# UM-Applied-Algorithms-Lab/AWRY

Hardware: AMD Instinct MI355X
Metric: k-mer count queries/sec (parallel_count, random 31-mers, index resident in HBM) (higher is better)
Workload: dtype u64

## Files before the change

### awry_amd/csrc/kernels_nt2_kmer.hip.h

```cpp
#pragma once

namespace awry {

__device__ __forceinline__ void tally_flush(unsigned long long* __restrict__ tally, uint32_t t_probe, uint32_t t_step, uint32_t t_blk) {
  atomicAdd(&tally[0], (unsigned long long)t_probe);
  atomicAdd(&tally[1], (unsigned long long)t_step);
  atomicAdd(&tally[2], (unsigned long long)t_blk);
}

template <bool USE_SEED, bool TALLY>
__global__ __launch_bounds__(256) void count_nt2_quad_kernel(DevIndex ix, const uint64_t* __restrict__ queries, uint64_t n, int L,
                                                             uint64_t* __restrict__ counts, unsigned long long* __restrict__ tally) {
  const int l = threadIdx.x & 3;
  const uint64_t nquads = ((uint64_t)gridDim.x * blockDim.x) >> 2;
  uint64_t q = ((uint64_t)blockIdx.x * blockDim.x + threadIdx.x) >> 2;
  const uint64_t* __restrict__ blocks = ix.blocks;
  const SeedEntry* __restrict__ seed = ix.seed;
  const int k = USE_SEED ? ix.seed_k : 1;
  const uint32_t cA = (uint32_t)ix.prefix_sums[1], cC = (uint32_t)ix.prefix_sums[2], cG = (uint32_t)ix.prefix_sums[3],
                 cN = (uint32_t)ix.prefix_sums[4], cT = (uint32_t)ix.prefix_sums[5], cEnd = (uint32_t)ix.prefix_sums[6];

  bool have = q < n;
  uint64_t w = have ? queries[q] : 0;
  bool fresh = true;
  uint32_t sp = 1, ep = 0;
  int i = 0;
  uint32_t t_probe = 0, t_step = 0, t_blk = 0;

  while (__any(have)) {
    if (have) {
      if (fresh) {
        if (USE_SEED) {
          const uint64_t sidx = ((w >> (2 * (L - k))) & ((1ull << (2 * k)) - 1));
          kmer_seed_start(seed[sidx], w, L - k, ix.seed_pos, sp, ep, i);
          if (TALLY) t_probe++;
        }
        if (!USE_SEED || i < 0) {
          const uint32_t c = (uint32_t)(w >> (2 * (L - 1))) & 3u;
          sp = c == 0 ? cA : (c == 1 ? cC : (c == 2 ? cG : cT));
          ep = (c == 0 ? cC : (c == 1 ? cG : (c == 2 ? cN : cEnd))) - 1;
          i = L - 1;
        }
        fresh = false;
      } else {
        i--;
        const uint32_t c = (uint32_t)(w >> (2 * i)) & 3u;
        const uint32_t cl = c == 0 ? cA : (c == 1 ? cC : (c == 2 ? cG : cT));
        if (TALLY) { t_step++; t_blk += ((sp - 1) >> 8) == (ep >> 8) ? 1u : 2u; }
        quad_step(blocks, cl, sp, ep, c, l);
      }
      if (sp > ep || i == 0) {
        if (l == 0) counts[q] = sp > ep ? 0ull : (uint64_t)(ep - sp) + 1ull;
        q += nquads;
        have = q < n;
        if (have) w = queries[q];
        fresh = true;
      }
    }
  }
  if (TALLY && l == 0) {
    tally_flush(tally, t_probe, t_step, t_blk);
  }
}

constexpr int TALLY_DEEP_STEP = 10;

template <bool USE_SEED, bool TALLY, bool VERIFY>
__global__ __launch_bounds__(256) void count_nt2_quad4_kernel(DevIndex ix, const uint64_t* __restrict__ queries, uint64_t n, int L,
                                                              uint64_t* __restrict__ counts, unsigned long long* __restrict__ tally) {
  const int lane = threadIdx.x & 63, l = lane & 3;
  const uint64_t nquads = ((uint64_t)gridDim.x * blockDim.x) >> 2;
  const uint64_t ngroups = (n + 3) >> 2;
  uint64_t m = ((uint64_t)blockIdx.x * blockDim.x + threadIdx.x) >> 2;
  const uint64_t* __restrict__ blocks = ix.blocks;
  const SeedEntry* __restrict__ seed = ix.seed;
  const int k = USE_SEED ? ix.seed_k : 1;
  const int verify_after = (int)ix.verify_after;
  const uint32_t cA = (uint32_t)ix.prefix_sums[1], cC = (uint32_t)ix.prefix_sums[2], cG = (uint32_t)ix.prefix_sums[3],
                 cN = (uint32_t)ix.prefix_sums[4], cT = (uint32_t)ix.prefix_sums[5], cEnd = (uint32_t)ix.prefix_sums[6];
  const int kshift = 2 * (L - k);
  const uint64_t kmask = (1ull << (2 * k)) - 1;
  bool have = m < ngroups;
  uint64_t wq = (have && 4 * m + l < n) ? queries[4 * m + l] : 0;
  uint64_t eq = 0;
  if (USE_SEED && have) { const SeedEntry e0 = seed[((wq >> kshift) & kmask)]; eq = (uint64_t)e0.sp | ((uint64_t)e0.cnt << 32); }
  uint64_t wq_next = (m + nquads < ngroups && 4 * (m + nquads) + l < n) ? queries[4 * (m + nquads) + l] : 0;
  int nvalid = have ? (int)(n - 4 * m < 4 ? n - 4 * m : 4) : 0;
  int t = 0;
  bool fresh = true;
  uint64_t w = 0, res = 0;
  uint32_t sp = 1, ep = 0;
  int i = 0, steps_done = 0;
  int mode = 0, vj = 0;
  uint32_t vhits = 0, vp = 0;
  uint32_t t_probe = 0, t_step = 0, t_blk = 0, t_vsa = 0, t_vtxt = 0, t_deep = 0;

  while (__any(have)) {
    if (have) {
      bool finished = false;
      uint64_t out_count = 0;
      if (!VERIFY || mode == 0) {
        if (fresh) {
          w = __shfl(wq, (lane & ~3) | t, 64);
          if (USE_SEED) {
            const uint64_t ev = __shfl(eq, (lane & ~3) | t, 64);
            kmer_seed_start(SeedEntry{(uint32_t)ev, (uint32_t)(ev >> 32)}, w, L - k, ix.seed_pos, sp, ep, i);
            if (TALLY) t_probe++;
          }
          if (!USE_SEED || i < 0) {
            const uint32_t c = (uint32_t)(w >> (2 * (L - 1))) & 3u;
            sp = c == 0 ? cA : (c == 1 ? cC : (c == 2 ? cG : cT));
            ep = (c == 0 ? cC : (c == 1 ? cG : (c == 2 ? cN : cEnd))) - 1;
            i = L - 1;
          }
          steps_done = 0;
          fresh = false;
        } else {
          i--;
          const uint32_t c = (uint32_t)(w >> (2 * i)) & 3u;
          const uint32_t cl = c == 0 ? cA : (c == 1 ? cC : (c == 2 ? cG : cT));
          if (TALLY) {
            const uint32_t nb = ((sp - 1) >> 8) == (ep >> 8) ? 1u : 2u;
            t_step++;
            t_blk += nb;
            if (steps_done >= TALLY_DEEP_STEP) t_deep += nb;
          }
          quad_step(blocks, cl, sp, ep, c, l);
          steps_done++;
        }
        if (sp > ep || i == 0) {
          finished = true;
          out_count = sp > ep ? 0ull : (uint64_t)(ep - sp) + 1ull;
        } else if (VERIFY) {
          const uint32_t cnt = ep - sp + 1u;
          if (verify_now(cnt, i, steps_done, verify_after)) { mode = 1; vj = 0; vhits = 0; }
        }
      } else if (mode == 1) {
        vp = ix.dense_sa[sp + (uint32_t)vj];
        if (TALLY) t_vsa++;
        if (vp >= (uint32_t)i) mode = 2;
        else vj++;
      } else {
        const uint32_t bad = quad_sum(verify_part(ix.text4, (uint64_t)vp - (uint64_t)i, i, 0, l, w));
        if (TALLY) t_vtxt++;
        if (!bad) vhits++;
        vj++;
        mode = 1;
      }
      if (VERIFY && mode == 1 && vj > (int)(ep - sp)) { finished = true; out_count = vhits; }
      if (finished) {
        if (l == t) res = out_count;
        t++;
        fresh = true;
        mode = 0;
        if (t == nvalid) {
          if (l < nvalid) counts[4 * m + l] = res;
          m += nquads;
          have = m < ngroups;
          t = 0;
          nvalid = have ? (int)(n - 4 * m < 4 ? n - 4 * m : 4) : 0;
          wq = wq_next;
          if (USE_SEED && have) { const SeedEntry e0 = seed[((wq >> kshift) & kmask)]; eq = (uint64_t)e0.sp | ((uint64_t)e0.cnt << 32); }
          wq_next = (m + nquads < ngroups && 4 * (m + nquads) + l < n) ? queries[4 * (m + nquads) + l] : 0;
        }
      }
    }
  }
  if (TALLY && l == 0) {
    tally_flush(tally, t_probe, t_step, t_blk);
    atomicAdd(&tally[5], (unsigned long long)t_deep);
    if (VERIFY) {
      atomicAdd(&tally[3], (unsigned long long)t_vsa);
      atomicAdd(&tally[4], (unsigned long long)t_vtxt);
    }
  }
}

constexpr int VMULTI = 4;
constexpr int LCX_LANE_ROWS = 4;
constexpr int LCX_TAIL_MAX = 16;

struct Nt2Survivors {
  uint64_t* w;
  uint64_t* range;
  uint32_t* q;
  uint32_t* count;
  uint64_t cap;
  uint32_t* lf_count = nullptr;
};

template <bool TALLY, bool VERIFY>
__device__ __forceinline__ unsigned probe_block(const DevIndex& ix, const uint64_t* __restrict__ queries, uint64_t n, int L,
                                                uint64_t* __restrict__ counts, const Nt2Survivors& sv,
                                                unsigned long long* __restrict__ tally) {
  __shared__ unsigned int s_count;
  constexpr int VQ = 192;
  __shared__ uint64_t s_vw[VERIFY ? 4 : 1][VQ];
  __shared__ uint32_t s_vsp[VERIFY ? 4 : 1][VQ];
  __shared__ uint32_t s_vq[VERIFY ? 4 : 1][VQ];
  __shared__ uint8_t s_vn[VERIFY ? 4 : 1][VQ];
  if (threadIdx.x == 0) s_count = 0;
  if (blockIdx.x == 0 && threadIdx.x == 0 && sv.lf_count) *sv.lf_count = 0;
  __syncthreads();
  const int lane = threadIdx.x & 63, wv_id = threadIdx.x >> 6;
  const SeedEntry* __restrict__ seed = ix.seed;
  const int k = ix.seed_k, i0 = L - k, kshift = 2 * (L - k);
  const uint64_t kmask = (1ull << (2 * k)) - 1;
  const uint64_t stride = (uint64_t)gridDim.x * blockDim.x;
  const uint64_t lane_lt = (1ull << lane) - 1;
  const uint64_t region = (uint64_t)blockIdx.x * sv.cap;
  const bool pos = VERIFY && ix.seed_pos;
  const int cx = (int)ix.ctx_extra, clen = SEED_CTX_LEN + cx;
  const bool verify = VERIFY && (i0 >= 3 || (pos && i0 >= 1));
  const bool lcx = VERIFY && ix.lcx_key != nullptr && i0 >= 1;
  int vcount = 0;
  uint32_t t_vsa = 0, t_vtxt = 0, t_lcx = 0;
  auto drain = [&](int base, int cnt) {
    uint64_t w[2];
    uint32_t q[2], sp[2], nc[2], vp[2];
    bool on[2];
#pragma unroll
    for (int h = 0; h < 2; h++) {
      const int s = base + lane + 64 * h;
      on[h] = lane + 64 * h < cnt;
      w[h] = on[h] ? s_vw[VERIFY ? wv_id : 0][s] : 0;
      q[h] = on[h] ? s_vq[VERIFY ? wv_id : 0][s] : 0;
      sp[h] = on[h] ? s_vsp[VERIFY ? wv_id : 0][s] : 0;
      nc[h] = on[h] ? s_vn[VERIFY ? wv_id : 0][s] : 0;
      vp[h] = sp[h];
      if (on[h] && !(nc[h] & 0x80u) && !(pos && nc[h] == 1u)) { vp[h] = ix.dense_sa[sp[h]]; if (TALLY) t_vsa++; }
    }
#pragma unroll
    for (int h = 0; h < 2; h++) {
      if (!on[h]) continue;
      uint64_t value = 0;
      if (nc[h] & 0x80u) {
        const uint64_t want = (w[h] & ((1ull << (2 * i0)) - 1)) << (64 - 2 * i0);
        const uint32_t rows = nc[h] & 0x7Fu;
        const uint64_t* __restrict__ kp = ix.lcx_key + sp[h];
        const uint64_t k0 = kp[0], k1 = kp[1], k2 = rows > 2u ? kp[2] : ~want, k3 = rows > 3u ? kp[3] : ~want;
        const int sh = 64 - 2 * i0;
        value = (((k0 ^ want) >> sh) == 0) + (((k1 ^ want) >> sh) == 0) + (((k2 ^ want) >> sh) == 0) + (((k3 ^ want) >> sh) == 0);
        if (TALLY) t_lcx++;
        counts[q[h]] = value;
        continue;
      }
      for (uint32_t c = 0; c < nc[h]; c++) {
        const uint32_t p = c ? ix.dense_sa[sp[h] + c] : vp[h];
        if (TALLY && c) t_vsa++;
        if (p >= (uint32_t)i0) {
          if (TALLY) t_vtxt++;
          value += verify_part(ix.text4, (uint64_t)p - (uint64_t)i0, i0, 0, 0, w[h]) ? 0ull : 1ull;
        }
      }
      counts[q[h]] = value;
    }
  };
  constexpr int NQ = 4;
  for (uint64_t wbase = (uint64_t)blockIdx.x * blockDim.x + (threadIdx.x & ~63u); wbase < n; wbase += NQ * stride) {
    uint64_t qv[NQ], wv[NQ];
    SeedEntry ev[NQ];
#pragma unroll
    for (int h = 0; h < NQ; h++) {
      qv[h] = wbase + lane + (uint64_t)h * stride;
      wv[h] = qv[h] < n ? queries[qv[h]] : 0;
    }
#pragma unroll
    for (int h = 0; h < NQ; h++) {
      ev[h] = SeedEntry{1u, 0u};
      if (qv[h] < n) ev[h] = seed_probe(seed + ((wv[h] >> kshift) & kmask));
    }
#pragma unroll
    for (int h = 0; h < NQ; h++) {
      const bool valid = qv[h] < n;
      const uint64_t q = qv[h], w = wv[h];
      const SeedEntry e = ev[h];
      const uint32_t cnt = seed_cnt(e);
      bool survivor = false, queued = false, lcx_q = false;
      uint64_t value = 0;
      if (valid) {
        if (cnt == SEED_CNT_SAT) survivor = true;
        else if (cnt == 0u) value = 0;
        else if (i0 == 0) value = cnt;
        else if (cnt == 1u && pos && seed_has_ctx(e) && i0 <= clen) {
          value = (w & ((1ull << (2 * i0)) - 1)) == (seed_full_ctx(e, cx) >> (2 * (clen - i0))) ? 1ull : 0ull;
        } else if (cnt == 1u && pos && seed_has_ctx(e)) {
          queued = ((w >> (2 * (i0 - clen))) & ((1ull << (2 * clen)) - 1)) == seed_full_ctx(e, cx);
        } else if (cnt == 1u) {
          const uint32_t nc = (uint32_t)(w >> (2 * (i0 - 1))) & 3u;
          survivor = seed_sym(e) == (int)(nc == 3u ? 5u : nc + 1u);
          if (verify && survivor) { queued = true; survivor = false; }
        } else if (lcx && !(e.cnt & (SEED_LCX_NONE | SEED_LCX_TAIL)) && cnt <= (uint32_t)LCX_LANE_ROWS) {
          queued = true;
          lcx_q = true;
        } else if (lcx && !(e.cnt & SEED_LCX_NONE)) {
          survivor = true;
        } else if (verify && cnt <= (uint32_t)VMULTI && (int)(3u * cnt) <= i0 + 2) {
          queued = true;
        } else survivor = true;
        if (!queued) counts[q] = value;
      }
      if (VERIFY) {
        const uint64_t qm = __ballot(queued);
        if (qm) {
          if (queued) {
            const int s = vcount + (int)__popcll(qm & lane_lt);
            s_vw[wv_id][s] = w;
            s_vsp[wv_id][s] = cnt == 1u && pos ? seed_position(e, cx) : e.sp;
            s_vq[wv_id][s] = (uint32_t)q;
            s_vn[wv_id][s] = (uint8_t)(cnt | (lcx_q ? 0x80u : 0u));
          }
          vcount += (int)__popcll(qm);
          __builtin_amdgcn_wave_barrier();
          if (vcount >= 128) {
            vcount -= 128;
            drain(vcount, 128);
            __builtin_amdgcn_wave_barrier();
          }
        }
      }
      const uint64_t sm = __ballot(survivor);
      if (sm) {
        unsigned int slot0 = 0;
        if (lane == 0) slot0 = atomicAdd(&s_count, (unsigned int)__popcll(sm));
        slot0 = __shfl(slot0, 0, 64);
        if (survivor) {
          const uint64_t s = region + slot0 + (uint64_t)__popcll(sm & lane_lt);
          sv.w[s] = w;
          sv.range[s] = (uint64_t)e.sp | ((uint64_t)(cnt | (e.cnt & (SEED_LCX_NONE | SEED_LCX_TAIL))) << 32);
          sv.q[s] = (uint32_t)q;
        }
      }
    }
  }
  if (VERIFY && vcount > 0) drain(0, vcount);
  if (TALLY) {
    if (blockIdx.x == 0 && threadIdx.x == 0) atomicAdd(&tally[0], (unsigned long long)n);
    if (VERIFY && (t_vsa | t_vtxt | t_lcx)) {
      atomicAdd(&tally[3], (unsigned long long)t_vsa);
      atomicAdd(&tally[4], (unsigned long long)t_vtxt);
      atomicAdd(&tally[6], (unsigned long long)t_lcx);
    }
  }
  __syncthreads();
  return s_count;
}

template <bool TALLY, bool VERIFY>
__global__ __launch_bounds__(256) void count_nt2_probe_kernel(DevIndex ix, const uint64_t* __restrict__ queries, uint64_t n, int L,
                                                              uint64_t* __restrict__ counts, Nt2Survivors sv,
                                                              unsigned long long* __restrict__ tally) {
  const unsigned ns = probe_block<TALLY, VERIFY>(ix, queries, n, L, counts, sv, tally);
  if (threadIdx.x == 0) sv.count[blockIdx.x] = ns;
}

template <bool TALLY, bool VERIFY, bool TABLE = false>
__device__ __forceinline__ void resume_block_list(const DevIndex& ix, const Nt2Survivors& sv, uint64_t region, uint64_t ns, int L,
                                                  uint64_t* __restrict__ counts, unsigned long long* __restrict__ tally, bool allow_lcx,
                                                  uint64_t r_start, uint64_t r_stride) {
  const int l = threadIdx.x & 3;
  uint64_t r = r_start;
  const uint64_t* __restrict__ blocks = ix.blocks;
  const int k = ix.seed_k;
  const int verify_after = (int)ix.verify_after;
  const bool lcx = VERIFY && ix.lcx_key != nullptr && allow_lcx;
  const uint32_t cA = (uint32_t)ix.prefix_sums[1], cC = (uint32_t)ix.prefix_sums[2], cG = (uint32_t)ix.prefix_sums[3],
                 cN = (uint32_t)ix.prefix_sums[4], cT = (uint32_t)ix.prefix_sums[5], cEnd = (uint32_t)ix.prefix_sums[6];
  bool have = r < ns, fresh = true;
  uint64_t w = 0;
  uint32_t sp = 1, ep = 0, qidx = 0;
  int i = 0, steps_done = 0;
  int mode = 0, vj = 0;
  uint32_t vhits = 0, vp = 0;
  uint32_t ub_a = 0, ub_b = 0;
  const LcxRefs lq{vp, vhits, ub_a, ub_b, vj};
  uint32_t t_step = 0, t_blk = 0, t_vsa = 0, t_vtxt = 0, t_lcx = 0, t_rp = 0;
  uint64_t nx_w = 0, nx_rg = 0;
  uint32_t nx_q = 0;
  if (have) { nx_w = sv.w[region + r]; nx_rg = sv.range[region + r]; nx_q = sv.q[region + r]; }
  while (__any(have)) {
    if (have) {
      bool finished = false;
      uint64_t out_count = 0;
      if (mode == 0) {
        if (fresh) {
          w = nx_w;
          const uint64_t rg = nx_rg;
          qidx = nx_q;
          if (r + r_stride < ns) { nx_w = sv.w[region + r + r_stride]; nx_rg = sv.range[region + r + r_stride]; nx_q = sv.q[region + r + r_stride]; }
          const uint32_t cf = (uint32_t)(rg >> 32), cnt = cf & SEED_CNT_SAT;
          steps_done = 0;
          fresh = false;
          if (qidx == 0xFFFFFFFFu) {
            sp = 1u; ep = 0u; i = 0;
          } else if (cnt == SEED_CNT_SAT) {
            const uint32_t c = (uint32_t)(w >> (2 * (L - 1))) & 3u;
            sp = c == 0 ? cA : (c == 1 ? cC : (c == 2 ? cG : cT));
            ep = (c == 0 ? cC : (c == 1 ? cG : (c == 2 ? cN : cEnd))) - 1;
            i = L - 1;
          } else {
            sp = (uint32_t)rg;
            ep = sp + cnt - 1u;
            i = L - k;
            if (lcx && cnt >= 2u && !(cf & SEED_LCX_NONE) && i > 0) {
              steps_done = 0;
              if (cf & SEED_LCX_TAIL) mode = 3;
              else { vp = ub_a = sp; vhits = ub_b = sp + cnt; vj = lcx_top_level(sp, cnt); mode = 4; }
              if (TABLE && ix.kmer_tab && cnt > (uint32_t)LCX_LANE_ROWS) { steps_done = mode; mode = 7; }
            }
          }
        }
        if (mode == 0) {
          const bool skip_step = VERIFY && i > 0 && sp <= ep && verify_now(ep - sp + 1u, i, steps_done, verify_after);
          if (i > 0 && sp <= ep && !skip_step) {
            i--;
            const uint32_t c = (uint32_t)(w >> (2 * i)) & 3u;
            const uint32_t cl = c == 0 ? cA : (c == 1 ? cC : (c == 2 ? cG : cT));
            if (TALLY) { t_step++; t_blk += ((sp - 1) >> 8) == (ep >> 8) ? 1u : 2u; }
            quad_step(blocks, cl, sp, ep, c, l);
            steps_done++;
          }
          if (sp > ep || i == 0) {
            finished = true;
            out_count = sp > ep ? 0ull : (uint64_t)(ep - sp) + 1ull;
          } else if (VERIFY) {
            const uint32_t cnt = ep - sp + 1u;
            if (verify_now(cnt, i, steps_done, verify_after)) { mode = 1; vj = 0; vhits = 0; }
          }
        }
      } else if (mode == 1) {
        vp = ix.dense_sa[sp + (uint32_t)vj];
        if (TALLY) t_vsa++;
        if (vp >= (uint32_t)i) mode = 2;
        else vj++;
      } else if (mode == 2) {
        const uint32_t bad = quad_sum(verify_part(ix.text4, (uint64_t)vp - (uint64_t)i, i, 0, l, w));
        if (TALLY) t_vtxt++;
        if (!bad) vhits++;
        vj++;
        mode = 1;
      } else if (mode == 3) {
        const uint32_t inc = (uint32_t)ix.lcx_key[ep];
        if (TALLY) t_lcx++;
        if (inc > (uint32_t)LCX_TAIL_MAX) { mode = 0; steps_done = 0; }
        else {
          const uint32_t nc = ep - sp + 1u - inc;
          steps_done = (int)inc;
          vp = ub_a = sp; vhits = ub_b = sp + nc; vj = nc ? lcx_top_level(sp, nc) : -1;
          mode = 4;
        }
      } else if (mode == 4) {
        uint64_t qlo, qhi;
        lcx_thresholds(w, i, &qlo, &qhi);
        const int lines = lcx_quad_step(ix, lq, qlo, qhi, l);
        if (TALLY) t_lcx += (uint32_t)lines;
        if (vj < 0) {
          vhits = ub_a - vp;
          if (steps_done) { mode = 5; vj = 0; }
          else { finished = true; out_count = vhits; }
        }
      } else if (mode == 5) {
        vp = (uint32_t)ix.lcx_rowpos[ep + 1u - (uint32_t)steps_done + (uint32_t)vj];
        if (TALLY) t_rp++;
        if (vp >= (uint32_t)i) mode = 6;
        else vj++;
      } else if (TABLE && mode == 7) {
        const uint64_t mx = kt_mix(w, L);
        const ulonglong2* p = reinterpret_cast<const ulonglong2*>(ix.kmer_tab + ((mx & ((1ull << ix.kmer_tab_bits) - 1)) << 4) + 4 * l);
        const ulonglong2 x = p[0], y = p[1];
        const uint64_t tag = mx >> ix.kmer_tab_bits;
        const uint64_t want = tag >= KT_TAG_NONE ? ~0ull : tag << KT_TAG_SHIFT;
        uint32_t c = l == 0 ? ((uint32_t)x.x >> KT_CNT_BITS & 1u) << 24 : 0u;
        c += ((x.x ^ want) >> KT_TAG_SHIFT) == 0 ? (uint32_t)x.x & (uint32_t)KT_CNT_MASK : 0u;
        c += ((x.y ^ want) >> KT_TAG_SHIFT) == 0 ? (uint32_t)x.y & (uint32_t)KT_CNT_MASK : 0u;
        c += ((y.x ^ want) >> KT_TAG_SHIFT) == 0 ? (uint32_t)y.x & (uint32_t)KT_CNT_MASK : 0u;
        c += ((y.y ^ want) >> KT_TAG_SHIFT) == 0 ? (uint32_t)y.y & (uint32_t)KT_CNT_MASK : 0u;
        c = quad_sum(c);
        if (TALLY) t_lcx++;
        const uint32_t found = c & 0xFFFFFFu;
        if (found == (uint32_t)KT_ASK || (found == 0u && (c >> 24))) {
          mode = steps_done;
          steps_done = 0;
        } else { finished = true; out_count = found; steps_done = 0; }
      } else {
        const uint32_t bad = quad_sum(verify_part(ix.text4, (uint64_t)vp - (uint64_t)i, i, 0, l, w));
        if (TALLY) t_vtxt++;
        if (!bad) vhits++;
        vj++;
        mode = 5;
      }
      if (VERIFY && mode == 1 && vj > (int)(ep - sp)) { finished = true; out_count = vhits; }
      if (mode == 5 && vj >= steps_done) { finished = true; out_count = vhits; }
      if (finished) {
        if (l == 0 && qidx != 0xFFFFFFFFu) counts[qidx] = out_count;
        r += r_stride;
        have = r < ns;
        fresh = true;
        mode = 0;
      }
    }
  }
  if (TALLY && l == 0) {
    atomicAdd(&tally[1], (unsigned long long)t_step);
    atomicAdd(&tally[2], (unsigned long long)t_blk);
    if (VERIFY) {
      atomicAdd(&tally[3], (unsigned long long)t_vsa);
      atomicAdd(&tally[4], (unsigned long long)t_vtxt);
      atomicAdd(&tally[6], (unsigned long long)t_lcx);
      atomicAdd(&tally[7], (unsigned long long)t_rp);
    }
  }
}

template <bool TALLY, bool VERIFY>
__global__ __launch_bounds__(256) void count_nt2_resume_kernel(DevIndex ix, Nt2Survivors sv, int L, uint64_t* __restrict__ counts,
                                                               unsigned long long* __restrict__ tally) {
  resume_block_list<TALLY, VERIFY>(ix, sv, (uint64_t)blockIdx.x * sv.cap, (uint64_t)sv.count[blockIdx.x], L, counts, tally, true, threadIdx.x >> 2, 64);
}

template <bool TALLY, bool VERIFY>
__global__ __launch_bounds__(256) void count_nt2_probe_resume_kernel(DevIndex ix, const uint64_t* __restrict__ queries, uint64_t n, int L, uint64_t* __restrict__ counts,
                                   Nt2Survivors sv, unsigned long long* __restrict__ tally) {
  const unsigned ns = probe_block<TALLY, VERIFY>(ix, queries, n, L, counts, sv, tally);
  resume_block_list<TALLY, VERIFY, true>(ix, sv, (uint64_t)blockIdx.x * sv.cap, (uint64_t)ns, L, counts, tally, true, threadIdx.x >> 2, 64);
}
constexpr int NT2_CHUNK = 256;

template <bool USE_SEED, bool TALLY>
__global__ __launch_bounds__(256) void count_nt2_chunk_kernel(DevIndex ix, const uint64_t* __restrict__ queries, uint64_t n, int L,
                                                              uint64_t* __restrict__ counts, unsigned long long* __restrict__ chunk_counter,
                                                              unsigned long long* __restrict__ tally) {
  __shared__ uint64_t lds_all[4 * NT2_CHUNK];
  const int lane = threadIdx.x & 63, l = lane & 3;
  volatile uint64_t* lds = lds_all + (threadIdx.x >> 6) * NT2_CHUNK;
  const uint64_t* __restrict__ blocks = ix.blocks;
  const SeedEntry* __restrict__ seed = ix.seed;
  const int k = USE_SEED ? ix.seed_k : 1;
  const uint32_t cA = (uint32_t)ix.prefix_sums[1], cC = (uint32_t)ix.prefix_sums[2], cG = (uint32_t)ix.prefix_sums[3],
                 cN = (uint32_t)ix.prefix_sums[4], cT = (uint32_t)ix.prefix_sums[5], cEnd = (uint32_t)ix.prefix_sums[6];
  const uint64_t nchunks = (n + NT2_CHUNK - 1) / NT2_CHUNK;
  const uint64_t quad_lt = (1ull << (lane & ~3)) - 1;
  uint32_t t_probe = 0, t_step = 0, t_blk = 0;

  for (;;) {
    unsigned long long c = 0;
    if (lane == 0) c = atomicAdd(chunk_counter, 1ull);
    c = __shfl(c, 0, 64);
    if (c >= nchunks) break;
    const uint64_t base = c * NT2_CHUNK;
    const int cn = (int)(n - base < (uint64_t)NT2_CHUNK ? n - base : (uint64_t)NT2_CHUNK);
    for (int j = 0; j < NT2_CHUNK / 64; j++) {
      const int s = j * 64 + lane;
      lds[s] = s < cn ? queries[base + s] : 0ull;
    }
    int cursor = 0;
    bool have = false, fresh = true;
    int slot = 0, i = 0;
    uint64_t w = 0;
    uint32_t sp = 1, ep = 0;
    for (;;) {
      const uint64_t needy = __ballot(!have && l == 0);
      if (!have) {
        const int idx = cursor + (int)__popcll(needy & quad_lt);
        if (idx < cn) { have = true; fresh = true; slot = idx; w = lds[idx]; }
      }
      cursor += (int)__popcll(needy);
      if (!__any(have)) break;
      if (have) {
        if (fresh) {
          if (USE_SEED) {
            const uint64_t sidx = ((w >> (2 * (L - k))) & ((1ull << (2 * k)) - 1));
            const SeedEntry e = seed[sidx];
            const uint32_t scnt = seed_cnt(e);
            sp = scnt ? e.sp : 1u;
            ep = scnt ? e.sp + scnt - 1u : 0u;
            i = L - k;
            if (scnt == 1u && i > 0) {
              const uint32_t nc = (uint32_t)(w >> (2 * (i - 1))) & 3u;
              if (seed_sym(e) != (int)(nc == 3u ? 5u : nc + 1u)) { sp = 1u; ep = 0u; }
            }
            if (scnt == SEED_CNT_SAT || (ix.seed_pos && scnt == 1u && sp <= ep && i > 0)) i = -1;
            if (TALLY) t_probe++;
          }
          if (!USE_SEED || i < 0) {
            const uint32_t ch = (uint32_t)(w >> (2 * (L - 1))) & 3u;
            sp = ch == 0 ? cA : (ch == 1 ? cC : (ch == 2 ? cG : cT));
            ep = (ch == 0 ? cC : (ch == 1 ? cG : (ch == 2 ? cN : cEnd))) - 1;
            i = L - 1;
          }
          fresh = false;
        } else {
          i--;
          const uint32_t ch = (uint32_t)(w >> (2 * i)) & 3u;
          const uint32_t cl = ch == 0 ? cA : (ch == 1 ? cC : (ch == 2 ? cG : cT));
          if (TALLY) { t_step++; t_blk += ((sp - 1) >> 8) == (ep >> 8) ? 1u : 2u; }
          quad_step(blocks, cl, sp, ep, ch, l);
        }
        if (sp > ep || i == 0) {
          if (l == 0) lds[slot] = sp > ep ? 0ull : (uint64_t)(ep - sp) + 1ull;
          have = false;
        }
      }
    }
    for (int j = 0; j < NT2_CHUNK / 64; j++) {
      const int s = j * 64 + lane;
      if (s < cn) counts[base + s] = lds[s];
    }
  }
  if (TALLY && l == 0) {
    tally_flush(tally, t_probe, t_step, t_blk);
  }
}

}
```

Baseline: 39.25 billion.

## Move k-mer table lookups to a lane-per-query pass before quad resume

Replaces the quad-cooperative mode-7 hash-table lookup inside the resume loop with a separate per-wavefront pass where each lane handles one survivor, probes the table with early exit, writes counts directly, and compacts the remaining survivors in place with ballot/popcount. The resume loop then processes each wave's compacted sublist with a per-wave stride of 16 quads and uses relaxed atomic loads to read freshly written records. This aims to reduce divergence and quad-lane waste on table hits and to shrink the list the slower FM-step/verify path must walk. It adds a block barrier and partitions survivors statically per wave, which may cause load imbalance.

```diff
diff --git a/awry_amd/csrc/kernels_nt2_kmer.hip.h b/awry_amd/csrc/kernels_nt2_kmer.hip.h
--- a/awry_amd/csrc/kernels_nt2_kmer.hip.h
+++ b/awry_amd/csrc/kernels_nt2_kmer.hip.h
@@ -354,7 +354,71 @@
   if (threadIdx.x == 0) sv.count[blockIdx.x] = ns;
 }
 
-template <bool TALLY, bool VERIFY, bool TABLE = false>
+template <bool FRESH, typename T>
+__device__ __forceinline__ T sv_record(const T* p) {
+  if constexpr (FRESH) return __hip_atomic_load(p, __ATOMIC_RELAXED, __HIP_MEMORY_SCOPE_AGENT);
+  else return *p;
+}
+
+template <bool TALLY>
+__device__ __forceinline__ uint32_t table_lane_pass(const DevIndex& ix, const Nt2Survivors& sv, uint64_t region, uint32_t ns, int L,
+                                                    uint64_t* __restrict__ counts, unsigned long long* __restrict__ tally, uint32_t* first) {
+  const int lane = threadIdx.x & 63;
+  const int wv_id = __builtin_amdgcn_readfirstlane((int)(threadIdx.x >> 6));
+  const uint32_t per = (ns + 3u) >> 2;
+  const uint32_t lo = min((uint32_t)wv_id * per, ns), hi = min(lo + per, ns);
+  const uint64_t lane_lt = (1ull << lane) - 1;
+  const int i0 = L - ix.seed_k;
+  const bool covered = ix.lcx_key != nullptr && i0 > 0;
+  const uint32_t bits = ix.kmer_tab_bits;
+  uint32_t wpos = lo, t_ask = 0;
+  uint64_t nx_w = 0, nx_rg = 0;
+  uint32_t nx_q = 0;
+  if (lo + lane < hi) { nx_w = sv.w[region + lo + lane]; nx_rg = sv.range[region + lo + lane]; nx_q = sv.q[region + lo + lane]; }
+  for (uint32_t base = lo; base < hi; base += 64u) {
+    const bool valid = base + lane < hi;
+    const uint64_t w = nx_w, rg = nx_rg;
+    const uint32_t q = nx_q;
+    if (base + 64u + lane < hi) { nx_w = sv.w[region + base + 64u + lane]; nx_rg = sv.range[region + base + 64u + lane]; nx_q = sv.q[region + base + 64u + lane]; }
+    const uint32_t cf = (uint32_t)(rg >> 32), cnt = cf & SEED_CNT_SAT;
+    const bool ask = valid && covered && q != 0xFFFFFFFFu && cnt != SEED_CNT_SAT && cnt > (uint32_t)LCX_LANE_ROWS && !(cf & SEED_LCX_NONE);
+    bool left = valid && !ask;
+    if (ask) {
+      const uint64_t mx = kt_mix(w, L);
+      const ulonglong2* __restrict__ p = reinterpret_cast<const ulonglong2*>(ix.kmer_tab + ((mx & ((1ull << bits) - 1)) << 4));
+      const uint64_t tag = mx >> bits;
+      const uint64_t want = tag >= KT_TAG_NONE ? ~0ull : tag << KT_TAG_SHIFT;
+      uint32_t found = 0;
+      bool done = false;
+      auto look = [&](uint64_t e) {
+        const uint32_t c = (uint32_t)e & (uint32_t)KT_CNT_MASK;
+        if (!done && (c == 0u || ((e ^ want) >> KT_TAG_SHIFT) == 0)) { found = c; done = true; }
+      };
+      bool marked = false;
+      for (int u = 0; u < 8 && !done; u += 2) {
+        const ulonglong2 x = p[u], y = p[u + 1];
+        if (u == 0) marked = (x.x & KT_OVERFLOW) != 0;
+        look(x.x); look(x.y); look(y.x); look(y.y);
+      }
+      if (found == (uint32_t)KT_ASK || (found == 0u && marked)) left = true;
+      else counts[q] = found;
+    }
+    if (TALLY) t_ask += (uint32_t)__popcll(__ballot(ask));
+    const uint64_t lm = __ballot(left);
+    if (left) {
+      const uint64_t s = region + wpos + (uint64_t)__popcll(lm & lane_lt);
+      sv.w[s] = w;
+      sv.range[s] = rg;
+      sv.q[s] = q;
+    }
+    wpos += (uint32_t)__popcll(lm);
+  }
+  if (TALLY && lane == 0 && t_ask) atomicAdd(&tally[6], (unsigned long long)t_ask);
+  *first = lo;
+  return wpos - lo;
+}
+
+template <bool TALLY, bool VERIFY, bool FRESH = false>
 __device__ __forceinline__ void resume_block_list(const DevIndex& ix, const Nt2Survivors& sv, uint64_t region, uint64_t ns, int L,
                                                   uint64_t* __restrict__ counts, unsigned long long* __restrict__ tally, bool allow_lcx,
                                                   uint64_t r_start, uint64_t r_stride) {
@@ -377,7 +441,7 @@
   uint32_t t_step = 0, t_blk = 0, t_vsa = 0, t_vtxt = 0, t_lcx = 0, t_rp = 0;
   uint64_t nx_w = 0, nx_rg = 0;
   uint32_t nx_q = 0;
-  if (have) { nx_w = sv.w[region + r]; nx_rg = sv.range[region + r]; nx_q = sv.q[region + r]; }
+  if (have) { nx_w = sv_record<FRESH>(&sv.w[region + r]); nx_rg = sv_record<FRESH>(&sv.range[region + r]); nx_q = sv_record<FRESH>(&sv.q[region + r]); }
   while (__any(have)) {
     if (have) {
       bool finished = false;
@@ -387,7 +451,11 @@
           w = nx_w;
           const uint64_t rg = nx_rg;
           qidx = nx_q;
-          if (r + r_stride < ns) { nx_w = sv.w[region + r + r_stride]; nx_rg = sv.range[region + r + r_stride]; nx_q = sv.q[region + r + r_stride]; }
+          if (r + r_stride < ns) {
+            nx_w = sv_record<FRESH>(&sv.w[region + r + r_stride]);
+            nx_rg = sv_record<FRESH>(&sv.range[region + r + r_stride]);
+            nx_q = sv_record<FRESH>(&sv.q[region + r + r_stride]);
+          }
           const uint32_t cf = (uint32_t)(rg >> 32), cnt = cf & SEED_CNT_SAT;
           steps_done = 0;
           fresh = false;
@@ -406,7 +474,6 @@
               steps_done = 0;
               if (cf & SEED_LCX_TAIL) mode = 3;
               else { vp = ub_a = sp; vhits = ub_b = sp + cnt; vj = lcx_top_level(sp, cnt); mode = 4; }
-              if (TABLE && ix.kmer_tab && cnt > (uint32_t)LCX_LANE_ROWS) { steps_done = mode; mode = 7; }
             }
           }
         }
@@ -464,24 +531,6 @@
         if (TALLY) t_rp++;
         if (vp >= (uint32_t)i) mode = 6;
         else vj++;
-      } else if (TABLE && mode == 7) {
-        const uint64_t mx = kt_mix(w, L);
-        const ulonglong2* p = reinterpret_cast<const ulonglong2*>(ix.kmer_tab + ((mx & ((1ull << ix.kmer_tab_bits) - 1)) << 4) + 4 * l);
-        const ulonglong2 x = p[0], y = p[1];
-        const uint64_t tag = mx >> ix.kmer_tab_bits;
-        const uint64_t want = tag >= KT_TAG_NONE ? ~0ull : tag << KT_TAG_SHIFT;
-        uint32_t c = l == 0 ? ((uint32_t)x.x >> KT_CNT_BITS & 1u) << 24 : 0u;
-        c += ((x.x ^ want) >> KT_TAG_SHIFT) == 0 ? (uint32_t)x.x & (uint32_t)KT_CNT_MASK : 0u;
-        c += ((x.y ^ want) >> KT_TAG_SHIFT) == 0 ? (uint32_t)x.y & (uint32_t)KT_CNT_MASK : 0u;
-        c += ((y.x ^ want) >> KT_TAG_SHIFT) == 0 ? (uint32_t)y.x & (uint32_t)KT_CNT_MASK : 0u;
-        c += ((y.y ^ want) >> KT_TAG_SHIFT) == 0 ? (uint32_t)y.y & (uint32_t)KT_CNT_MASK : 0u;
-        c = quad_sum(c);
-        if (TALLY) t_lcx++;
-        const uint32_t found = c & 0xFFFFFFu;
-        if (found == (uint32_t)KT_ASK || (found == 0u && (c >> 24))) {
-          mode = steps_done;
-          steps_done = 0;
-        } else { finished = true; out_count = found; steps_done = 0; }
       } else {
         const uint32_t bad = quad_sum(verify_part(ix.text4, (uint64_t)vp - (uint64_t)i, i, 0, l, w));
         if (TALLY) t_vtxt++;
@@ -521,8 +570,18 @@
 template <bool TALLY, bool VERIFY>
 __global__ __launch_bounds__(256) void count_nt2_probe_resume_kernel(DevIndex ix, const uint64_t* __restrict__ queries, uint64_t n, int L, uint64_t* __restrict__ counts,
                                    Nt2Survivors sv, unsigned long long* __restrict__ tally) {
-  const unsigned ns = probe_block<TALLY, VERIFY>(ix, queries, n, L, counts, sv, tally);
-  resume_block_list<TALLY, VERIFY, true>(ix, sv, (uint64_t)blockIdx.x * sv.cap, (uint64_t)ns, L, counts, tally, true, threadIdx.x >> 2, 64);
+  const unsigned ns = __builtin_amdgcn_readfirstlane(probe_block<TALLY, VERIFY>(ix, queries, n, L, counts, sv, tally));
+  uint64_t region = (uint64_t)blockIdx.x * sv.cap;
+  uint32_t left = ns, r_start = threadIdx.x >> 2, r_stride = 64;
+  if (VERIFY && ix.kmer_tab) {
+    uint32_t first = 0;
+    left = table_lane_pass<TALLY>(ix, sv, region, ns, L, counts, tally, &first);
+    region += first;
+    r_start &= 15u;
+    r_stride = 16;
+    __syncthreads();
+  }
+  resume_block_list<TALLY, VERIFY, true>(ix, sv, region, left, L, counts, tally, true, r_start, r_stride);
 }
 constexpr int NT2_CHUNK = 256;
 
```

New measurement: 38.90 billion. No clear change (-0.9%).
